# massquantity/LibRecommender

Hardware: AMD Instinct MI355X
Metric: train samples/sec (higher is better)
Workload: dtype f32 (split-bf16 x6 MFMA products, f32 accumulate); 1 GPU; DeepFM ranking train step, 1M users x 1M items x 200 sparse fields (10,000,200 sparse rows), embed_size=64, hidden=(128,64,32), Zipf(1.05) ids; per_gpu_batch=16384, global_batch=16384, fields=202, embed_size=64, table_rows=12000202, parallelism=single, launch=one hipGraph replay per step

## Files before the change

### include/libreco_hip.h

```cpp
#ifndef LIBRECO_HIP_H_
#define LIBRECO_HIP_H_

#include <stddef.h>
#include <stdint.h>

#ifdef __cplusplus
extern "C" {
#endif

#define LR_OK 0
#define LR_EINVAL (-1)
#define LR_ESHAPE (-2)
#define LR_EWORKSPACE (-3)

typedef void* lr_stream_t;

const char* lr_strerror(int code);
int lr_abi_version(void);
int lr_graph_foreign_nodes(void* graph, int* n_nodes_out);

int lr_embed_gather_f32(const float* table, int64_t V, int K, const int32_t* idx,
                        int64_t n, float* out, lr_stream_t stream);

#define LR_COMBINER_SUM 0
// ... 199 lines not shown
                                float momentum, const float* gamma, const float* beta,
                                float* moving_mean, float* moving_var, float* mean, float* inv, float* s,
                                float* t, lr_stream_t stream);
int lr_deepfm_l1_fold_stats_bias_f32(const float* partial, int F, int C, int K, int64_t B, float eps,
                                     float momentum, const float* gamma, const float* beta,
                                     float* moving_mean, float* moving_var, float* mean, float* inv, float* s,
                                     float* t, const float* W, const float* b, int H1, float* bias_partial,
                                     lr_stream_t stream);
int lr_deepfm_l1_pack_scaled_f32(const float* W, const float* scale, int F, int K, int H1, float* WpA,
                                 float* WpB, const float* red_partial, int red_nblk, float* red_out,
                                 lr_stream_t stream);
int lr_deepfm_l1_fold_bias_slabs(int n_rows);
int lr_deepfm_l1_fold_bias_f32(const float* t, const float* W, const float* b, int n_rows, int H1,
                               float* partial, lr_stream_t stream);
int lr_deepfm_l1_fold_bwd_f32(const float* part, int n_slabs, int n_rows, int H1, int64_t B,
                              const float* sgz, const float* W, const float* gamma, const float* beta,
                              const float* mean, const float* inv, float* dW, float* dgamma,
                              float* dbeta, float* db, float* bn_a, float* bn_c, lr_stream_t stream);

size_t lr_adam_coef_bytes(void);
int lr_adam_coef_store(lr_adam_hp hp, void* coef_dev, lr_stream_t stream);
int lr_adam_dense_dc_f32(float* table, float* m, float* v, int64_t n, const float* grad,
                         const void* coef_dev, lr_stream_t stream);
int lr_fm_rows_adam_dc_f32(float* table, float* m, float* v, float* lin, float* lin_m, float* lin_v,
                           int64_t V, int K, const float* ge, const float* gl, const float* wp,
                           const float* bn_a, const float* bn_c, const float* lin_scale, int64_t B,
                           int F, const int32_t* seg_pos, const int32_t* seg_rows,
                           const int32_t* seg_start, const int32_t* n_seg, const void* coef_dev,
                           void* ws, size_t ws_bytes, lr_stream_t stream);
int lr_embed_scatter_adam_dc_f32(float* table, float* m, float* v, int64_t V, int K, const float* grad,
                                 const int32_t* seg_pos, const int32_t* seg_rows, const int32_t* seg_start,
                                 const int32_t* n_seg, int64_t n_max, const void* coef_dev,
                                 void* ws, size_t ws_bytes, lr_stream_t stream);
int lr_embed_scatter_adam_lin_dc_f32(float* table, float* m, float* v, int64_t V, int K, const float* grad,
                                     float* lin, float* lin_m, float* lin_v, const float* glin,
                                     const int32_t* seg_pos, const int32_t* seg_rows,
                                     const int32_t* seg_start, const int32_t* n_seg, int64_t n_max,
                                     const void* coef_dev, lr_stream_t stream);

int lr_table_colstats_f32(const float* table, int64_t V, int K, const int32_t* idx, int64_t B, int F, int C,
                          float* partial, lr_stream_t stream);
int lr_bn_remainder_f32(float* G, const float* x, const float* a, const float* c, int64_t rows,
                        int64_t rows_per_plane, int64_t period, int Kp, lr_stream_t stream);

size_t lr_segments_fields_ws_bytes(int64_t B, int F);
int lr_segments_build_fields(const int32_t* idxT, int64_t B, int F, const int32_t* field_row_start,
                             int32_t* seg_pos, int32_t* seg_rows, int32_t* seg_start,
                             int32_t* n_seg, int32_t* slotT, void* ws, size_t ws_bytes,
                             lr_stream_t stream);
int lr_segments_build_fields_runs(const int32_t* idxT, int64_t B, int F, const int32_t* field_row_start,
                                  int32_t* seg_pos, int32_t* seg_rows, int32_t* seg_start,
                                  int32_t* n_seg, int32_t* slotT, int32_t* runT, void* ws, size_t ws_bytes,
                                  lr_stream_t stream);

size_t lr_owner_partition_ws_bytes(int64_t n_max, int W);
int lr_owner_partition_i32(const int32_t* rows, const int32_t* n_seg, int64_t n_max, int W, int32_t* perm,
                           int32_t* send_ids, int64_t* counts, void* ws, size_t ws_bytes, lr_stream_t stream);

size_t lr_din_attn_ws_bytes(int64_t B, int L, int K, int H);
int lr_din_attn_path(int K, int L, int backward);
int lr_din_build_ids_i32(const int32_t* users, const int32_t* items, const int32_t* sparse, int sparse_ld,
                         const int32_t* cols, int n_plain, const int32_t* seqs, const int32_t* lens, int64_t B, int L,
                         int32_t user_off, int32_t item_off, int32_t sparse_off, int32_t* ids, lr_stream_t stream);
int lr_din_attn_pool_fwd_f32(const float* item_table, int64_t V, int K,
                             const int32_t* item, const int32_t* seq, const int32_t* len,
                             int64_t B, int L, const float* W1, const float* b1,
                             const float* W2, const float* b2, int H, float* out,
                             float* attn, float* hid , int32_t* order_out ,
                             lr_stream_t stream);
int lr_din_attn_pool_bwd_f32(const float* item_table, int64_t V, int K,
                             const int32_t* item, const int32_t* seq, const int32_t* len,
                             int64_t B, int L, const float* W1, const float* b1,
                             const float* W2, const float* b2, int H, const float* attn,
                             const float* gout, float* gq, float* gkey, float* gW1,
                             float* gb1, float* gW2, float* gb2, void* ws, size_t ws_bytes,
                             lr_stream_t stream);
int lr_din_attn_pool_bwd_parts_f32(const float* item_table, int64_t V, int K,
                                   const int32_t* item, const int32_t* seq, const int32_t* len,
                                   int64_t B, int L, const float* W1, const float* b1,
                                   const float* W2, const float* b2, int H, const float* attn,
                                   const float* gout, float* gq, float* gkey, float* gW1,
                                   float* gb1, float* gW2, float* gb2, void* ws, size_t ws_bytes,
                                   int parts, int keep_pad_rows, const float* hid ,
                                   const int32_t* order , lr_stream_t stream);
int lr_din_attn_dense_fwd_f32(const float* q, const float* keys, int K, const int32_t* len,
                              int64_t B, int L, const float* W1, const float* b1,
                              const float* W2, const float* b2, int H, float* out,
                              float* attn, lr_stream_t stream);
int lr_din_attn_dense_bwd_f32(const float* q, const float* keys, int K, const int32_t* len,
                              int64_t B, int L, const float* W1, const float* b1,
                              const float* W2, const float* b2, int H, const float* attn,
                              const float* gout, float* gq, float* gkey, float* gW1,
                              float* gb1, float* gW2, float* gb2, void* ws, size_t ws_bytes,
                              lr_stream_t stream);

void lr_score_topk_test_mute(int ut);
size_t lr_score_topk_ws_bytes(int64_t B, int64_t N, int D, int k);
int lr_score_topk_f32(const float* users, int64_t B, const float* items, int64_t N, int D,
                      const int64_t* consumed_ptr ,
                      const int32_t* consumed_idx, const uint8_t* filter_flag ,
                      int k, int64_t item_base, float* out_scores ,
                      int64_t* out_ids , void* ws, size_t ws_bytes,
                      lr_stream_t stream);
int lr_score_topk_sb_f32(const float* users, int64_t B, const float* items, int64_t N, int D,
                         const int64_t* consumed_ptr, const int32_t* consumed_idx, const uint8_t* filter_flag,
                         int k, int64_t item_base, float* out_scores, int64_t* out_ids, void* ws, size_t ws_bytes,
// ... 323 lines not shown
```

### librecommender_amd/_lib.py

```python
from __future__ import annotations

import ctypes as C
import os
from pathlib import Path

LIB_PATH = Path(__file__).resolve().parent / "lib" / "liblibreco_hip.so"

LR_OK, LR_EINVAL, LR_ESHAPE, LR_EWORKSPACE = 0, -1, -2, -3
ABI_VERSION = 25

COMBINERS = {"sum": 0, "mean": 1, "sqrtn": 2}


class AdamHP(C.Structure):

    _fields_ = [
        ("lr", C.c_double),
        ("beta1", C.c_double),
        ("beta2", C.c_double),
        ("eps", C.c_double),
        ("weight_decay", C.c_double),
        ("step", C.c_int32),
        ("tf_style", C.c_int32),
    ]
# ... 82 lines not shown
                                    _i64, _p, _p, _p, _p, _u32, _f32, _int, _p]),
    "lr_mlp_first_bwd_f32": (_int, [_p, _p, _p, _p, _p, _p, _p, _i64, _int, _p, _p, _p]),
    "lr_reduce_partials_f32": (_int, [_p, _int, _i64, _i64, _p, _p]),
    "lr_deepfm_l1_fold_stats_f32": (_int, [_p, _int, _int, _int, _i64, _f32, _f32, _p, _p, _p, _p, _p, _p, _p, _p, _p]),
    "lr_deepfm_l1_pack_scaled_f32": (_int, [_p, _p, _int, _int, _int, _p, _p, _p, _int, _p, _p]),
    "lr_deepfm_l1_fold_stats_bias_f32": (_int, [_p, _int, _int, _int, _i64, _f32, _f32, _p, _p, _p, _p, _p, _p, _p, _p, _p, _p, _int,
                                                _p, _p]),
    "lr_deepfm_l1_fold_bias_slabs": (_int, [_int]),
    "lr_deepfm_l1_fold_bias_f32": (_int, [_p, _p, _p, _int, _int, _p, _p]),
    "lr_deepfm_l1_fold_bwd_f32": (_int, [_p, _int, _int, _int, _i64, _p, _p, _p, _p, _p, _p, _p, _p, _p, _p, _p, _p, _p]),
    "lr_fm_field_stats_slots_f32": (_int, [_p, _int, _p, _p, _p, _p, _int, _int, _p, _p, _p, _p]),
    "lr_fm_rows_grad_f32": (_int, [_p, _p, _i64, _int, _p, _p, _p, _p, _p, _p, _i64, _int, _p, _p, _p, _p, _p, _p, _p, _p,
                                   _sz, _p]),
    "lr_fm_rows_grad_compact_f32": (_int, [_p, _p, _i64, _int, _p, _p, _p, _p, _p, _p, _i64, _int, _p, _p, _p, _p, _p, _p, _p,
                                           _sz, _p]),
    "lr_adam_dense_rows_f32": (_int, [_p, _p, _p, _p, _p, _p, _i64, _int, _p, _p, _p, _p, _i64, _p, AdamHP, _p]),
    "lr_adam_dense_rows_dc_f32": (_int, [_p, _p, _p, _p, _p, _p, _i64, _int, _p, _p, _p, _p, _i64, _p, _p, _p]),
    "lr_spmm_csr_ws_bytes": (_sz, [_i64, _i64, _int]),
    "lr_spmm_csr_bucketed_f32": (_int, [_p, _p, _p, _i64, _i64, _p, _int, _p, _p, _p, _sz, _int, _p]),
    "lr_spmm_csr_masked_f32": (_int, [_p, _p, _p, _i64, _i64, _p, _int, _p, _p, _p, _p, _p, _sz, _int, _p]),
    "lr_bitmap_ids_i32": (_int, [_p, _i64, _i64, _p, _int, _p]),
    "lr_row_slots_i32": (_int, [_p, _p, _i64, _p, _int, _p]),
    "lr_spmm_csr_adam_f32": (_int, [_p, _p, _p, _i64, _i64, _p, _int, _p, _p, _p, _p, _p, _p, _f32, AdamHP, _p, _sz, _int, _p]),
    "lr_din_build_ids_i32": (_int, [_p, _p, _p, _int, _p, _int, _p, _p, _i64, _int, _int, _int, _int, _p, _p]),
    "lr_softmax_ce_supported": (_int, [_i64, _i64, _int]),
    "lr_softmax_ce_fwd_ws_bytes": (_sz, [_i64, _i64, _int, _int]),
    "lr_softmax_ce_fwd_f32": (_int, [_p, _i64, _p, _i64, _int, _p, _p, _p, _i64, _p, _p, _p, _p, _sz, _int, _p]),
    "lr_softmax_ce_bwd_cols_f32": (_int, [_p, _i64, _p, _i64, _int, _p, _p, _p, _i64, _p, _p, _p, _int, _p]),
    "lr_reduce_job_bytes": (_sz, []),
    "lr_reduce_partials_multi_f32": (_int, [_p, _int, _i64, _p]),
    "lr_pair_mlp_supported": (_int, [_int, _int]),
    "lr_pair_mlp_f32": (_int, [_p, _i64, _p, _i64, _int, _p, _p, _int, _p, _f32, _p, _i64, _int, _p]),
    "lr_pair_mlp_sb_f32": (_int, [_p, _i64, _p, _i64, _int, _p, _p, _int, _p, _f32, _p, _i64, _int, _p]),
    "lr_score_topk_test_mute": (None, [_int]),
    "lr_mfma_f32_probe": (_int, [_int, _int, _p, _p]),
    "lr_probe_occupy": (_int, [_int, _sz, _i64, _p]),
    "lr_clock_probe": (_int, [_p, _p]),
    "lr_clock_probe_slots": (_int, []),
    "lr_mlp_tail3_resident_blocks": (_int, []),
    "lr_adam_coef_bytes": (_sz, []),
    "lr_adam_coef_store": (_int, [AdamHP, _p, _p]),
    "lr_adam_dense_dc_f32": (_int, [_p, _p, _p, _i64, _p, _p, _p]),
    "lr_fm_rows_adam_dc_f32": (_int, [_p, _p, _p, _p, _p, _p, _i64, _int, _p, _p, _p, _p, _p, _p, _i64,
                                      _int, _p, _p, _p, _p, _p, _p, _sz, _p]),
    "lr_embed_scatter_adam_dc_f32": (_int, [_p, _p, _p, _i64, _int, _p, _p, _p, _p, _p, _i64, _p, _p, _sz, _p]),
    "lr_embed_scatter_adam_lin_dc_f32": (_int, [_p, _p, _p, _i64, _int, _p, _p, _p, _p, _p, _p, _p, _p, _p, _i64, _p, _p]),
    "lr_table_colstats_f32": (_int, [_p, _i64, _int, _p, _i64, _int, _int, _p, _p]),
    "lr_bn_remainder_f32": (_int, [_p, _p, _p, _p, _i64, _i64, _i64, _int, _p]),
    "lr_csr_laplacian_ws_bytes": (_sz, [_i64]),
    "lr_csr_laplacian_build": (_int, [_p, _p, _i64, _i64, _i64, _p, _p, _p, _p, _p, _p, _sz, _p]),
    "lr_segments_fields_ws_bytes": (_sz, [_i64, _int]),
    "lr_segments_build_fields": (_int, [_p, _i64, _int, _p, _p, _p, _p, _p, _p, _p, _sz, _p]),
    "lr_segments_build_fields_runs": (_int, [_p, _i64, _int, _p, _p, _p, _p, _p, _p, _p, _p, _sz, _p]),
    "lr_owner_partition_ws_bytes": (_sz, [_i64, _int]),
    "lr_owner_partition_i32": (_int, [_p, _p, _i64, _int, _p, _p, _p, _p, _sz, _p]),
    "lr_din_attn_ws_bytes": (_sz, [_i64, _int, _int, _int]),
    "lr_din_attn_path": (_int, [_int, _int, _int]),
    "lr_din_attn_pool_fwd_f32": (_int, [_p, _i64, _int, _p, _p, _p, _i64, _int, _p, _p, _p, _p,
                                        _int, _p, _p, _p, _p, _p]),
    "lr_din_attn_pool_bwd_f32": (_int, [_p, _i64, _int, _p, _p, _p, _i64, _int, _p, _p, _p, _p,
                                        _int, _p, _p, _p, _p, _p, _p, _p, _p, _p, _sz, _p]),
    "lr_din_attn_pool_bwd_parts_f32": (_int, [_p, _i64, _int, _p, _p, _p, _i64, _int, _p, _p, _p, _p,
                                              _int, _p, _p, _p, _p, _p, _p, _p, _p, _p, _sz, _int, _int, _p, _p, _p]),
    "lr_din_attn_dense_fwd_f32": (_int, [_p, _p, _int, _p, _i64, _int, _p, _p, _p, _p, _int, _p,
                                         _p, _p]),
    "lr_din_attn_dense_bwd_f32": (_int, [_p, _p, _int, _p, _i64, _int, _p, _p, _p, _p, _int, _p,
                                         _p, _p, _p, _p, _p, _p, _p, _p, _sz, _p]),
    "lr_score_topk_ws_bytes": (_sz, [_i64, _i64, _int, _int]),
    "lr_score_topk_f32": (_int, [_p, _i64, _p, _i64, _int, _p, _p, _p, _int, _i64, _p, _p, _p,
                                 _sz, _p]),
    "lr_score_topk_sb_f32": (_int, [_p, _i64, _p, _i64, _int, _p, _p, _p, _int, _i64, _p, _p, _p,
                                 _sz, _p]),
    "lr_score_topk_filter_kp": (_int, [_int]),
    "lr_score_topk_filter_ws_bytes": (_sz, [_i64, _i64, _int, _int]),
    "lr_score_topk_filter_f32": (_int, [_p, _i64, _p, _i64, _int, _p, _p, _p, _int, _i64, _p, _p, _p,
                                        _sz, _int, _int, _p, _p]),
    "lr_topk_merge_f32": (_int, [_p, _p, _int, _i64, _int, _p, _p, _p]),
    "lr_ivf_supported": (_int, [_i64, _i64, _int, _int, _int, _int]),
    "lr_ivf_search_ws_bytes": (_sz, [_i64, _i64, _int, _int, _int, _int]),
    "lr_ivf_build_ws_bytes": (_sz, [_i64, _int]),
    "lr_ivf_centroids_ws_bytes": (_sz, [_i64, _int]),
    "lr_ivf_assign_f32": (_int, [_p, _i64, _p, _int, _int, _p, _p, _p]),
    "lr_ivf_build_lists": (_int, [_p, _i64, _int, _p, _p, _p, _sz, _p]),
    "lr_ivf_centroids_f32": (_int, [_p, _i64, _int, _p, _p, _i64, _int, _p, _p, _sz, _p]),
    "lr_ivf_search_f32": (_int, [_p, _i64, _p, _int, _p, _p, _p, _i64, _int, _p, _p, _p, _int, _int, _p, _p, _p, _sz, _p]),
    "lr_spmm_csr_f32": (_int, [_p, _p, _p, _i64, _p, _int, _p, _p, _p]),
    "lr_pair_dot_f32": (_int, [_p, _i64, _p, _i64, _int, _p, _p, _i64, _p, _p]),
    "lr_als_supported": (_int, [_int]),
    "lr_als_plan_params": (_int, [_int, _p]),
    "lr_als_ws_bytes": (_sz, [_i64, _int]),
    "lr_als_gram_ws_bytes": (_sz, [_i64, _int]),
    "lr_als_gram_f32": (_int, [_p, _i64, _int, _f32, _int, _p, _p, _sz, _p]),
    "lr_als_half_sweep_f32": (_int, [_p, _p, _p, _i64, _p, _p, _int, _p, _int, _int, _int, _p, _i64, _i64, _i64, _i64,
                                     _p, _p, _sz, _int, _p]),
    "lr_cf_sim_tile_cols": (_int, []),
    "lr_cf_sim_ws_bytes": (_sz, []),
    "lr_cf_sim_f32": (_int, [_p, _p, _p, _p, _p, _p, _i64, _p, _p, _int, _int, _p, _p, _p, _i64, _int, _p, _p, _p, _p,
                             _p, _sz, _p]),
    "lr_cf_select_max": (_int, []),
    "lr_cf_topk_f32": (_int, [_p, _p, _p, _i64, _i64, _p, _p, _p, _p]),
    "lr_cf_recommend_ws_bytes": (_sz, [_i64, _i64]),
    "lr_cf_recommend_f32": (_int, [_p, _i64, _int, _p, _p, _p, _p, _p, _p, _i64, _i64, _p, _p, _int, _i64, _p, _p, _p,
                                   _p, _p, _p, _sz, _p]),
    "lr_cf_predict_f32": (_int, [_p, _p, _i64, _p, _p, _p, _p, _p, _p, _i64, _int, _f32, _f32, _f32, _p, _p, _p]),
    "lr_cf_pair_state_f32": (_int, [_p, _p, _p, _p, _p, _p, _i64, _p, _p, _p, _i64, _int, _p, _p, _p, _p, _p, _p, _sz, _p]),
    "lr_cf_sumsq_f32": (_int, [_p, _p, _i64, _int, _p, _p]),
# ... 144 lines not shown
```

### librecommender_amd/csrc/segments.hip

```cpp
#include <cstring>

#include <rocprim/rocprim.hpp>

#include "common.hpp"

namespace lr {

__global__ __launch_bounds__(kBlock) void seg_keys_kernel(const int32_t* __restrict__ idx,
                                                          int64_t n, uint32_t V,
                                                          uint32_t* __restrict__ keys) {
  const int64_t stride = static_cast<int64_t>(gridDim.x) * kBlock;
  for (int64_t i = static_cast<int64_t>(blockIdx.x) * kBlock + threadIdx.x; i < n; i += stride) {
    const int32_t id = idx[i];
    keys[i] = (id >= 0 && static_cast<uint32_t>(id) < V) ? static_cast<uint32_t>(id) : V;
  }
}

__global__ __launch_bounds__(kBlock) void seg_heads_kernel(const uint32_t* __restrict__ keys,
                                                           int64_t n, uint32_t V,
                                                           int32_t* __restrict__ heads,
                                                           int32_t* __restrict__ n_seg,
                                                           int32_t* __restrict__ seg_start) {
  const int64_t stride = static_cast<int64_t>(gridDim.x) * kBlock;
  const int64_t t0 = static_cast<int64_t>(blockIdx.x) * kBlock + threadIdx.x;
  if (t0 == 0) {
    n_seg[0] = 0;
    seg_start[0] = 0;
  }
  for (int64_t i = t0; i < n; i += stride) {
    const uint32_t k = keys[i];
    heads[i] = (k < V && (i == 0 || keys[i - 1] != k)) ? 1 : 0;
  }
}

__global__ __launch_bounds__(kBlock) void seg_emit_kernel(
    const uint32_t* __restrict__ keys, const int32_t* __restrict__ rank, int64_t n, uint32_t V,
    const int32_t* __restrict__ seg_pos, int32_t* __restrict__ seg_rows,
    int32_t* __restrict__ seg_start, int32_t* __restrict__ n_seg,
    int32_t* __restrict__ pos_to_seg) {
  const int64_t stride = static_cast<int64_t>(gridDim.x) * kBlock;
  for (int64_t i = static_cast<int64_t>(blockIdx.x) * kBlock + threadIdx.x; i < n; i += stride) {
    const uint32_t k = keys[i];
    if (k >= V) {
      if (pos_to_seg != nullptr) pos_to_seg[seg_pos[i]] = -1;
      continue;
    }
    const int32_t r = rank[i];
    if (pos_to_seg != nullptr) pos_to_seg[seg_pos[i]] = r - 1;
    if (i == 0 || keys[i - 1] != k) {
      seg_rows[r - 1] = static_cast<int32_t>(k);
      seg_start[r - 1] = static_cast<int32_t>(i);
    }
    if (i == n - 1 || keys[i + 1] >= V) {
      seg_start[r] = static_cast<int32_t>(i + 1);
      n_seg[0] = r;
    }
  }
}

static inline size_t align_up(size_t x, size_t a = 256) { return (x + a - 1) / a * a; }

static inline int key_bits(int64_t V) {
  int bits = 1;
  while (bits < 32 && (static_cast<uint64_t>(1) << bits) <= static_cast<uint64_t>(V)) ++bits;
  return bits;
}

struct SegWs {
  uint32_t* keys_in;
  uint32_t* keys_out;
  int32_t* rank;
  void* prim;
  size_t prim_bytes;
};

static inline size_t seg_fixed_bytes(int64_t n) {
  return align_up(static_cast<size_t>(n) * 4) * 3;
}

constexpr int kFS = 16384;
constexpr int kSortThreads = 1024;
constexpr int kSortWaves = kSortThreads / 64;
constexpr int kFSE = kFS / kSortThreads;
constexpr int kFSW = kFS / kSortWaves;
constexpr uint32_t kKeyInvalid = 0xFFFFFFFFu;

__device__ __forceinline__ uint64_t match_digit(uint32_t d) {
  uint64_t mask = ~0ull;
#pragma unroll
  for (int k = 0; k < 8; ++k) {
    const bool bit = (d >> k) & 1u;
    const uint64_t bk = __ballot(bit);
    mask &= bit ? bk : ~bk;
  }
  return mask;
}

__global__ __launch_bounds__(kSortThreads) void seg_field_sort_kernel(
    const int32_t* __restrict__ idxT, int B, const int32_t* __restrict__ frs,
    uint64_t* __restrict__ sorted, int32_t* __restrict__ fcount) {
  extern __shared__ __attribute__((aligned(16))) char smem[];
  uint64_t* buf = reinterpret_cast<uint64_t*>(smem);
  int* cnt = reinterpret_cast<int*>(buf + kFS);
  int* wsum = cnt + kSortWaves * 256;
  const int f = blockIdx.x;
  const int tid = threadIdx.x, wid = tid >> 6, lane = tid & 63;
  const int32_t lo = frs[f], hi = frs[f + 1];
  const uint64_t lt = (1ull << lane) - 1ull;
  const int32_t* col = idxT + static_cast<int64_t>(f) * B;
  int bits = 0;
  while (bits < 32 && ((1ull << bits) - 1ull) < static_cast<uint64_t>(hi > lo ? hi - lo : 0)) ++bits;
  const int n_pass = (bits + 7) / 8;

  uint64_t x[kFSE];
#pragma unroll
  for (int s = 0; s < kFSE; ++s) {
    const int p = wid * kFSW + s * 64 + lane;
    const int32_t id = p < B ? col[p] : -1;
    const bool ok = id >= lo && id < hi;
    const uint32_t key = ok ? static_cast<uint32_t>(id - lo) : kKeyInvalid;
    x[s] = (static_cast<uint64_t>(key) << 32) | static_cast<uint32_t>(p);
  }

  int* my = cnt + wid * 256;
  for (int pass = 0; pass < n_pass; ++pass) {
    const int shift = 32 + 8 * pass;
    for (int i = tid; i < kSortWaves * 256; i += kSortThreads) cnt[i] = 0;
    __syncthreads();
#pragma unroll
    for (int s = 0; s < kFSE; ++s) {
      const uint32_t d = static_cast<uint32_t>(x[s] >> shift) & 255u;
      const uint64_t mk = match_digit(d);
      if ((mk & lt) == 0ull)
        __hip_atomic_fetch_add(my + d, __popcll(mk), __ATOMIC_RELAXED, __HIP_MEMORY_SCOPE_WORKGROUP);
    }
    __syncthreads();
    int tot = 0, inc = 0;
    if (tid < 256) {
#pragma unroll
      for (int w = 0; w < kSortWaves; ++w) tot += cnt[w * 256 + tid];
      inc = tot;
#pragma unroll
      for (int o = 1; o < 64; o <<= 1) {
        const int y = __shfl_up(inc, o);
        if (lane >= o) inc += y;
      }
      if (lane == 63) wsum[wid] = inc;
    }
    __syncthreads();
    if (tid < 256) {
      int run = inc - tot;
      for (int w = 0; w < wid; ++w) run += wsum[w];
#pragma unroll
      for (int w = 0; w < kSortWaves; ++w) {
        const int c = cnt[w * 256 + tid];
        cnt[w * 256 + tid] = run;
        run += c;
      }
    }
    __syncthreads();
#pragma unroll
    for (int s = 0; s < kFSE; ++s) {
      uint32_t d = static_cast<uint32_t>(x[s] >> shift) & 255u;
      asm volatile("" : "+v"(d));
      const uint64_t mk = match_digit(d);
      const int leader = __ffsll(static_cast<long long>(mk)) - 1;
      int old = 0;
      if (lane == leader)
        old = __hip_atomic_fetch_add(my + d, __popcll(mk), __ATOMIC_RELAXED, __HIP_MEMORY_SCOPE_WORKGROUP);
      old = __shfl(old, leader);
      buf[old + __popcll(mk & lt)] = x[s];
      if ((s & 3) == 3) __builtin_amdgcn_sched_barrier(0);
    }
    __syncthreads();
#pragma unroll
    for (int s = 0; s < kFSE; ++s) x[s] = buf[wid * kFSW + s * 64 + lane];
  }
  if (n_pass == 0) {
#pragma unroll
    for (int s = 0; s < kFSE; ++s) buf[wid * kFSW + s * 64 + lane] = x[s];
  }
  __syncthreads();

  int nv = 0, nh = 0;
  uint64_t* dst = sorted + static_cast<int64_t>(f) * B;
#pragma unroll
  for (int s = 0; s < kFSE; ++s) {
    const int i = wid * kFSW + s * 64 + lane;
    const uint32_t key = static_cast<uint32_t>(x[s] >> 32);
    const bool valid = key != kKeyInvalid;
    const bool head = valid && (i == 0 || static_cast<uint32_t>(buf[i > 0 ? i - 1 : 0] >> 32) != key);
    nv += __popcll(__ballot(valid));
    nh += __popcll(__ballot(head));
    if (i < B) dst[i] = x[s];
  }
  __syncthreads();
  if (lane == 0) { wsum[wid * 2] = nv; wsum[wid * 2 + 1] = nh; }
  __syncthreads();
  if (tid == 0) {
    int tv = 0, th = 0;
    for (int w = 0; w < kSortWaves; ++w) { tv += wsum[2 * w]; th += wsum[2 * w + 1]; }
    fcount[2 * f] = tv;
    fcount[2 * f + 1] = th;
  }
}

constexpr int kEmitThreads = 1024;
constexpr int kEmitWaves = kEmitThreads / 64;

__global__ __launch_bounds__(kEmitThreads) void seg_field_emit_kernel(
    const uint64_t* __restrict__ sorted, const int32_t* __restrict__ fcount, int B, int F,
    const int32_t* __restrict__ frs, int32_t* __restrict__ seg_pos, int32_t* __restrict__ seg_rows,
    int32_t* __restrict__ seg_start, int32_t* __restrict__ n_seg, int32_t* __restrict__ slotT,
    int32_t* __restrict__ runT) {
  __shared__ int red[2][kEmitWaves];
  __shared__ int wh[kEmitWaves];
  const int f = blockIdx.x;
  const int tid = threadIdx.x, wid = tid >> 6, lane = tid & 63;
  const uint64_t lt = (1ull << lane) - 1ull;
  int bv = 0, bh = 0;
  for (int g = tid; g < f; g += kEmitThreads) { bv += fcount[2 * g]; bh += fcount[2 * g + 1]; }
#pragma unroll
  for (int o = 32; o > 0; o >>= 1) { bv += __shfl_xor(bv, o); bh += __shfl_xor(bh, o); }
  if (lane == 0) { red[0][wid] = bv; red[1][wid] = bh; }
  __syncthreads();
  int base_v = 0, base_h = 0;
#pragma unroll
  for (int w = 0; w < kEmitWaves; ++w) { base_v += red[0][w]; base_h += red[1][w]; }
  const int nv = fcount[2 * f];
  const int32_t lo = frs[f];
  const uint64_t* src = sorted + static_cast<int64_t>(f) * B;
  const int chunk = ((B + kEmitWaves - 1) / kEmitWaves + 63) / 64 * 64;
  const int i0 = wid * chunk, i1 = (i0 + chunk) < B ? (i0 + chunk) : B;
  auto is_head = [&](int i, uint32_t key) {
    return i < nv && (i == 0 || static_cast<uint32_t>(src[i - 1] >> 32) != key);
// ... 183 lines not shown
  const size_t a = align_up(static_cast<size_t>(n) * 4);
  SegWs w;
  w.keys_in = reinterpret_cast<uint32_t*>(p);
  w.keys_out = reinterpret_cast<uint32_t*>(p + a);
  w.rank = reinterpret_cast<int32_t*>(p + 2 * a);
  w.prim = p + 3 * a;
  w.prim_bytes = ws_bytes - 3 * a;

  const uint32_t Vu = static_cast<uint32_t>(V);
  const int grid = grid_for(n, kBlock);
  hipLaunchKernelGGL(seg_keys_kernel, dim3(grid), dim3(kBlock), 0, s, idx, n, Vu, w.keys_in);

  const int bits = key_bits(V);
  size_t need = 0;
  hipError_t e = hipSuccess;
  if (n <= kRsMaxN) {
    const size_t hist_bytes = align_up((static_cast<size_t>((n + kRsKPB - 1) / kRsKPB) + 1) * 256 * 4);
    if (hist_bytes + a > w.prim_bytes) return LR_EWORKSPACE;
    const int rc = own_radix_sort(w.keys_in, w.keys_out, seg_pos, reinterpret_cast<uint32_t*>(static_cast<char*>(w.prim) + hist_bytes),
                                  w.rank, static_cast<int32_t*>(w.prim), n, bits, s);
    if (rc != LR_OK) return rc;
  } else {
    rocprim::counting_iterator<int32_t> iota(0);
    e = rocprim::radix_sort_pairs(nullptr, need, w.keys_in, w.keys_out, iota, seg_pos, static_cast<size_t>(n), 0u,
                                  static_cast<unsigned>(bits), s);
    if (e != hipSuccess) return static_cast<int>(e);
    if (need > w.prim_bytes) return LR_EWORKSPACE;
    e = rocprim::radix_sort_pairs(w.prim, need, w.keys_in, w.keys_out, iota, seg_pos, static_cast<size_t>(n), 0u,
                                  static_cast<unsigned>(bits), s);
    if (e != hipSuccess) return static_cast<int>(e);
  }

  hipLaunchKernelGGL(seg_heads_kernel, dim3(grid), dim3(kBlock), 0, s, w.keys_out, n, Vu,
                     w.rank, n_seg, seg_start);
  need = 0;
  e = rocprim::inclusive_scan(nullptr, need, w.rank, w.rank, static_cast<size_t>(n),
                              rocprim::plus<int32_t>(), s);
  if (e != hipSuccess) return static_cast<int>(e);
  if (need > w.prim_bytes) return LR_EWORKSPACE;
  e = rocprim::inclusive_scan(w.prim, need, w.rank, w.rank, static_cast<size_t>(n),
                              rocprim::plus<int32_t>(), s);
  if (e != hipSuccess) return static_cast<int>(e);

  hipLaunchKernelGGL(seg_emit_kernel, dim3(grid), dim3(kBlock), 0, s, w.keys_out, w.rank, n,
                     Vu, seg_pos, seg_rows, seg_start, n_seg, pos_to_seg);
  return launch_status();
}

extern "C" size_t lr_segments_fields_ws_bytes(int64_t B, int F) {
  if (B < 0 || F < 1) return 0;
  return align_up(static_cast<size_t>(B) * F * 8) + align_up(static_cast<size_t>(F) * 8);
}

static int build_fields_impl(const int32_t* idxT, int64_t B, int F, const int32_t* field_row_start, int32_t* seg_pos,
                             int32_t* seg_rows, int32_t* seg_start, int32_t* n_seg, int32_t* slotT, int32_t* runT, void* ws,
                             size_t ws_bytes, lr_stream_t stream) {
  LR_CHECK_ARG(B >= 1 && F >= 1);
  LR_CHECK_ARG(idxT && field_row_start && seg_pos && seg_rows && seg_start && n_seg && ws);
  if (B > kFS || B * F >= (int64_t(1) << 31)) return LR_ESHAPE;
  if (ws_bytes < lr_segments_fields_ws_bytes(B, F)) return LR_EWORKSPACE;
  hipStream_t s = as_stream(stream);
  uint64_t* sorted = static_cast<uint64_t*>(ws);
  int32_t* fcount = reinterpret_cast<int32_t*>(static_cast<char*>(ws) + align_up(static_cast<size_t>(B) * F * 8));
  const size_t lds = static_cast<size_t>(kFS) * 8 + kSortWaves * 256 * 4 + kSortWaves * 2 * 4;
  static bool attr_set = false;
  if (!attr_set) {
    hipError_t e = hipFuncSetAttribute(reinterpret_cast<const void*>(seg_field_sort_kernel),
                                       hipFuncAttributeMaxDynamicSharedMemorySize, static_cast<int>(lds));
    if (e != hipSuccess) return static_cast<int>(e);
    attr_set = true;
  }
  hipLaunchKernelGGL(seg_field_sort_kernel, dim3(F), dim3(kSortThreads), lds, s, idxT, static_cast<int>(B),
                     field_row_start, sorted, fcount);
  hipLaunchKernelGGL(seg_field_emit_kernel, dim3(F), dim3(kEmitThreads), 0, s, sorted, fcount,
                     static_cast<int>(B), F, field_row_start, seg_pos, seg_rows, seg_start, n_seg, slotT, runT);
  return launch_status();
}

extern "C" int lr_segments_build_fields(const int32_t* idxT, int64_t B, int F, const int32_t* field_row_start,
                                        int32_t* seg_pos, int32_t* seg_rows, int32_t* seg_start, int32_t* n_seg,
                                        int32_t* slotT, void* ws, size_t ws_bytes, lr_stream_t stream) {
  return build_fields_impl(idxT, B, F, field_row_start, seg_pos, seg_rows, seg_start, n_seg, slotT, nullptr, ws, ws_bytes,
                           stream);
}

extern "C" int lr_segments_build_fields_runs(const int32_t* idxT, int64_t B, int F, const int32_t* field_row_start,
                                             int32_t* seg_pos, int32_t* seg_rows, int32_t* seg_start, int32_t* n_seg,
                                             int32_t* slotT, int32_t* runT, void* ws, size_t ws_bytes, lr_stream_t stream) {
  LR_CHECK_ARG(runT != nullptr);
  return build_fields_impl(idxT, B, F, field_row_start, seg_pos, seg_rows, seg_start, n_seg, slotT, runT, ws, ws_bytes,
                           stream);
}

constexpr int kOwnChunk = 1024;
constexpr int kOwnMaxW = 64;

template <bool kPlace>
__device__ __forceinline__ void owner_chunk(const int32_t* __restrict__ rows, int n, int W, int chunk, int (*cnt)[4][kOwnMaxW],
                                            int* my_owner, int* my_rank) {
  const int tid = threadIdx.x, wid = tid >> 6, lane = tid & 63;
  const uint64_t lt = (1ull << lane) - 1ull;
#pragma unroll
  for (int it = 0; it < 4; ++it) {
    const int i = chunk * kOwnChunk + it * kBlock + tid;
    const int o = i < n ? static_cast<int>(static_cast<uint32_t>(rows[i]) % static_cast<uint32_t>(W)) : -1;
    int rank = 0;
    for (int w = 0; w < W; ++w) {
      const uint64_t mk = __ballot(o == w);
      if (o == w) rank = __popcll(mk & lt);
      if (lane == 0) cnt[it][wid][w] = __popcll(mk);
    }
    if (kPlace) { my_owner[it] = o; my_rank[it] = rank; }
  }
}

__global__ __launch_bounds__(kBlock) void owner_count_kernel(const int32_t* __restrict__ rows, const int32_t* __restrict__ n_seg,
                                                             int W, int32_t* __restrict__ chunk_cnt) {
  __shared__ int cnt[4][4][kOwnMaxW];
  const int n = n_seg[0];
  const int chunk = blockIdx.x;
  if (chunk * kOwnChunk >= n) {
    for (int w = threadIdx.x; w < W; w += kBlock) chunk_cnt[static_cast<int64_t>(chunk) * W + w] = 0;
    return;
  }
  owner_chunk<false>(rows, n, W, chunk, cnt, nullptr, nullptr);
  __syncthreads();
  for (int w = threadIdx.x; w < W; w += kBlock) {
    int t = 0;
#pragma unroll
// ... 97 lines not shown
```

### librecommender_amd/ops.py

```python
from __future__ import annotations

import os

from dataclasses import dataclass
from typing import NamedTuple, Optional

import torch

from . import _lib
from ._lib import AdamHP, COMBINERS, check


def _stream() -> int:
    return torch.cuda.current_stream().cuda_stream


class KernelTimer:

    def __init__(self):
        self.names = set()
        self.events = {}

    def enable(self, *names):
        self.names = set(names)
# ... 138 lines not shown
        nbytes = _lib.load().lr_segments_ws_bytes(self.n_max, self.V)
        self.ws = torch.empty(nbytes, dtype=torch.uint8, device=device)
        self.pos = torch.empty(self.n_max, dtype=torch.int32, device=device)
        self.rows = torch.empty(self.n_max, dtype=torch.int32, device=device)
        self.start = torch.empty(self.n_max + 1, dtype=torch.int32, device=device)
        self.n_seg = torch.zeros(1, dtype=torch.int32, device=device)
        self.slots = None
        self._long_ws = {}

    def long_ws(self, K: int) -> torch.Tensor:
        ws = self._long_ws.get(K)
        if ws is None:
            ws = self._long_ws[K] = torch.empty(max(_lib.load().lr_embed_scatter_ws_bytes(self.n_max, K), 256),
                                                dtype=torch.uint8, device=self.device)
        return ws

    def hist_ws(self, K: int) -> torch.Tensor:
        ws = self._long_ws.get(("hist", K))
        if ws is None:
            ws = self._long_ws[("hist", K)] = torch.empty(max(_lib.load().lr_svdpp_hist_grad_ws_bytes(self.n_max, K), 256),
                                                          dtype=torch.uint8, device=self.device)
        return ws

    def ftrl_ws(self) -> torch.Tensor:
        ws = self._long_ws.get("ftrl")
        if ws is None:
            ws = self._long_ws["ftrl"] = torch.empty(max(_lib.load().lr_ftrl_rows_ws_bytes(self.n_max), 256),
                                                     dtype=torch.uint8, device=self.device)
        return ws

    def build(self, idx: torch.Tensor, want_slots: bool = False) -> Segments:
        _req(idx, torch.int32, "idx")
        n = idx.numel()
        if n > self.n_max:
            raise ValueError(f"idx has {n} entries, builder was sized for {self.n_max}")
        if want_slots and self.slots is None:
            self.slots = torch.empty(self.n_max, dtype=torch.int32, device=self.device)
        _call("lr_segments_build", _ptr(idx), n, self.V, _ptr(self.pos), _ptr(self.rows),
                                            _ptr(self.start), _ptr(self.n_seg),
                                            _ptr(self.slots) if want_slots else None, _ptr(self.ws),
                                            self.ws.numel(), _stream())
        seg = Segments(self.pos, self.rows, self.start, self.n_seg, n, self.V, owner=self)
        seg.slots = self.slots[:n] if want_slots else None
        return seg


def build_segments(idx: torch.Tensor, V: int) -> Segments:
    return SegmentBuilder(max(idx.numel(), 1), V, idx.device).build(idx)


class FieldSegmentBuilder:

    MAX_B = 16384

    def __init__(self, B_max: int, F: int, V: int, device: torch.device, want_runs: bool = False):
        self.B_max, self.F, self.V, self.device = int(B_max), int(F), int(V), device
        n = self.B_max * self.F
        self.ws = torch.empty(_lib.load().lr_segments_fields_ws_bytes(self.B_max, self.F), dtype=torch.uint8, device=device)
        self.pos = torch.empty(n, dtype=torch.int32, device=device)
        self.rows = torch.empty(n, dtype=torch.int32, device=device)
        self.start = torch.empty(n + 1, dtype=torch.int32, device=device)
        self.n_seg = torch.zeros(1, dtype=torch.int32, device=device)
        self.slotT = torch.empty((self.F, self.B_max), dtype=torch.int32, device=device)
        self.runT = torch.empty((self.F, self.B_max), dtype=torch.int32, device=device) if want_runs else None

    def build(self, idxT: torch.Tensor, field_row_start: torch.Tensor) -> Segments:
        _req(idxT, torch.int32, "idxT", 2)
        _req(field_row_start, torch.int32, "field_row_start", 1)
        F, B = idxT.shape
        if F != self.F or B > self.B_max or field_row_start.numel() != F + 1:
            raise ValueError("idxT does not match this builder")
        cut = (lambda t: t if B == self.B_max else t.view(-1)[: F * B].view(F, B))
        slotT = cut(self.slotT)
        seg = Segments(self.pos, self.rows, self.start, self.n_seg, B * F, self.V)
        if self.runT is None:
            _call("lr_segments_build_fields", _ptr(idxT), B, F, _ptr(field_row_start), _ptr(self.pos), _ptr(self.rows),
                  _ptr(self.start), _ptr(self.n_seg), _ptr(slotT), _ptr(self.ws), self.ws.numel(), _stream())
        else:
            seg.runT = cut(self.runT)
            _call("lr_segments_build_fields_runs", _ptr(idxT), B, F, _ptr(field_row_start), _ptr(self.pos), _ptr(self.rows),
                  _ptr(self.start), _ptr(self.n_seg), _ptr(slotT), _ptr(seg.runT), _ptr(self.ws), self.ws.numel(), _stream())
        seg.slotT = slotT
        return seg


class OwnerPartition:

    def __init__(self, n_max: int, W: int, device: torch.device):
        self.n_max, self.W = int(n_max), int(W)
        self.ws = torch.empty(max(_lib.load().lr_owner_partition_ws_bytes(self.n_max, self.W), 256), dtype=torch.uint8, device=device)
        self.perm = torch.empty(self.n_max, dtype=torch.int32, device=device)
        self.send_ids = torch.empty(self.n_max, dtype=torch.int32, device=device)
        self.counts = torch.zeros(self.W + 1, dtype=torch.int64, device=device)

    def run(self, rows: torch.Tensor, n_seg: torch.Tensor):
        _req(rows, torch.int32, "rows", 1)
        _req(n_seg, torch.int32, "n_seg", 1)
        if rows.numel() > self.n_max:
            raise ValueError("rows exceed this partition's capacity")
        _call("lr_owner_partition_i32", _ptr(rows), _ptr(n_seg), rows.numel(), self.W, _ptr(self.perm), _ptr(self.send_ids),
              _ptr(self.counts), _ptr(self.ws), self.ws.numel(), _stream())
        return self.perm, self.send_ids, self.counts


def idx_transpose(idx: torch.Tensor, out: Optional[torch.Tensor] = None) -> torch.Tensor:
    _req(idx, torch.int32, "idx", 2)
    B, F = idx.shape
    if out is None:
        out = torch.empty((F, B), dtype=torch.int32, device=idx.device)
    _call("lr_idx_transpose_i32", _ptr(idx), B, F, _ptr(out), _stream())
    return out


def din_build_ids(users, items, sparse, cols, seqs, lens, user_off: int, item_off: int, sparse_off: int,
                  out: torch.Tensor) -> torch.Tensor:
    for t_, n_ in ((users, "users"), (items, "items"), (seqs, "seqs"), (lens, "lens"), (out, "out")):
        _req(t_, torch.int32, n_)
    B, L = seqs.shape
    n_plain = 0
    if sparse is not None:
        _req(sparse, torch.int32, "sparse", 2)
        n_plain = int(cols.numel()) if cols is not None else sparse.shape[1]
        if cols is not None:
            _req(cols, torch.int32, "cols", 1)
    if out.numel() != (2 + n_plain + 2 + L) * B or not seqs.is_contiguous() or (sparse is not None and not sparse.is_contiguous()):
        raise ValueError("`out` must hold (2 + n_plain + 2 + L) * B ids; seqs / sparse contiguous")
    _call("lr_din_build_ids_i32", _ptr(users), _ptr(items), _ptr(sparse), sparse.shape[1] if sparse is not None else 0,
          _ptr(cols), n_plain, _ptr(seqs), _ptr(lens), B, L, int(user_off), int(item_off), int(sparse_off), _ptr(out), _stream())
    return out


def _din_order(order, B):
    if order is not None and (order.dtype != torch.int32 or not order.is_contiguous() or order.numel() != B):
        raise ValueError("order must be a contiguous int32 tensor of B elements")
    return order


def embed_segment_sum(grad: torch.Tensor, seg: Segments) -> torch.Tensor:
    _req(grad, torch.float32, "grad")
    K = grad.shape[-1]
    if grad.numel() != seg.n * K:
        raise ValueError("grad rows must match the segmented index count")
    grows = torch.zeros((max(seg.n, 1), K), dtype=torch.float32, device=grad.device)
    ws = seg.long_ws(K)
    _call("lr_embed_segment_sum_f32", _ptr(grad), K, _ptr(seg.pos), _ptr(seg.start), _ptr(seg.n_seg), seg.n, _ptr(grows),
          _ptr(ws), 0 if ws is None else ws.numel(), _stream())
    return grows


def embed_scatter_add(table: torch.Tensor, grad: torch.Tensor, seg: Segments, alpha: float = 1.0) -> None:
    _req(table, torch.float32, "table", 2)
    _req(grad, torch.float32, "grad")
    V, K = table.shape
    if grad.numel() != seg.n * K or V != seg.V:
        raise ValueError("shape mismatch")
    ws = seg.long_ws(K)
    _call("lr_embed_scatter_add_f32", _ptr(table), V, K, _ptr(grad), _ptr(seg.pos), _ptr(seg.rows), _ptr(seg.start),
          _ptr(seg.n_seg), seg.n, float(alpha), _ptr(ws), 0 if ws is None else ws.numel(), _stream())


def embed_scatter_adam(table: torch.Tensor, m: torch.Tensor, v: torch.Tensor, grad: torch.Tensor,
                       seg: Segments, hp) -> None:
# ... 2694 lines not shown
```

Before: 6.582 million samples/s.

## Fuse per-field counting into idx transpose and emit segments inside sort kernel

```diff
diff --git a/include/libreco_hip.h b/include/libreco_hip.h
--- a/include/libreco_hip.h
+++ b/include/libreco_hip.h
@@ -275,6 +275,8 @@
                                   int32_t* seg_pos, int32_t* seg_rows, int32_t* seg_start,
                                   int32_t* n_seg, int32_t* slotT, int32_t* runT, void* ws, size_t ws_bytes,
                                   lr_stream_t stream);
+int lr_idx_transpose_count_i32(const int32_t* idx, int64_t B, int F, const int32_t* field_row_start,
+                               int64_t max_field_rows, int32_t* idxT, void* ws, size_t ws_bytes, lr_stream_t stream);
 
 size_t lr_owner_partition_ws_bytes(int64_t n_max, int W);
 int lr_owner_partition_i32(const int32_t* rows, const int32_t* n_seg, int64_t n_max, int W, int32_t* perm,
diff --git a/librecommender_amd/_lib.py b/librecommender_amd/_lib.py
--- a/librecommender_amd/_lib.py
+++ b/librecommender_amd/_lib.py
@@ -158,6 +158,7 @@
     "lr_segments_fields_ws_bytes": (_sz, [_i64, _int]),
     "lr_segments_build_fields": (_int, [_p, _i64, _int, _p, _p, _p, _p, _p, _p, _p, _sz, _p]),
     "lr_segments_build_fields_runs": (_int, [_p, _i64, _int, _p, _p, _p, _p, _p, _p, _p, _p, _sz, _p]),
+    "lr_idx_transpose_count_i32": (_int, [_p, _i64, _int, _p, _i64, _p, _p, _sz, _p]),
     "lr_owner_partition_ws_bytes": (_sz, [_i64, _int]),
     "lr_owner_partition_i32": (_int, [_p, _p, _i64, _int, _p, _p, _p, _p, _sz, _p]),
     "lr_din_attn_ws_bytes": (_sz, [_i64, _int, _int, _int]),
diff --git a/librecommender_amd/csrc/segments.hip b/librecommender_amd/csrc/segments.hip
--- a/librecommender_amd/csrc/segments.hip
+++ b/librecommender_amd/csrc/segments.hip
@@ -1,4 +1,5 @@
 #include <cstring>
+#include <mutex>
 
 #include <rocprim/rocprim.hpp>
 
@@ -96,9 +97,59 @@
   return mask;
 }
 
+constexpr int kCountThreads = 1024;
+constexpr int kCountWaves = kCountThreads / 64;
+constexpr int64_t kCountMaxRows = (int64_t(160) * 1024 - 256) * 8;
+
+__global__ __launch_bounds__(kCountThreads) void seg_field_count_kernel(
+    const int32_t* __restrict__ idx, int B, int F, const int32_t* __restrict__ frs, uint32_t cap_rows,
+    int32_t* __restrict__ idxT, int32_t* __restrict__ fcount) {
+  extern __shared__ __attribute__((aligned(16))) char smem[];
+  uint32_t* bm = reinterpret_cast<uint32_t*>(smem);
+  __shared__ int red[2][kCountWaves];
+  const int per = (F + 7) / 8;
+  const int f = static_cast<int>(blockIdx.x % 8u) * per + static_cast<int>(blockIdx.x / 8u);
+  if (f >= F) return;
+  const int tid = threadIdx.x, wid = tid >> 6, lane = tid & 63;
+  const int32_t lo = frs[f], hi = frs[f + 1];
+  const uint32_t range = hi > lo ? static_cast<uint32_t>(hi - lo) : 0u;
+  const uint32_t rows = range < cap_rows ? range : cap_rows;
+  const int nwords = static_cast<int>((rows + 31u) / 32u);
+  for (int w = tid; w < nwords; w += kCountThreads) bm[w] = 0u;
+  __syncthreads();
+  int nv = 0;
+  int32_t* dst = idxT + static_cast<int64_t>(f) * B;
+  const int32_t* src = idx + f;
+#pragma unroll 4
+  for (int b = tid; b < B; b += kCountThreads) {
+    const int32_t id = src[static_cast<int64_t>(b) * F];
+    dst[b] = id;
+    const bool ok = id >= lo && id < hi;
+    nv += ok ? 1 : 0;
+    const uint32_t r = static_cast<uint32_t>(id - lo);
+    if (ok && r < rows) atomicOr(&bm[r >> 5], 1u << (r & 31u));
+  }
+  __syncthreads();
+  int nh = 0;
+  for (int w = tid; w < nwords; w += kCountThreads) nh += __popc(bm[w]);
+#pragma unroll
+  for (int o = 32; o > 0; o >>= 1) { nv += __shfl_xor(nv, o); nh += __shfl_xor(nh, o); }
+  if (lane == 0) { red[0][wid] = nv; red[1][wid] = nh; }
+  __syncthreads();
+  if (tid == 0) {
+    int tv = 0, th = 0;
+    for (int w = 0; w < kCountWaves; ++w) { tv += red[0][w]; th += red[1][w]; }
+    fcount[2 * f] = tv;
+    fcount[2 * f + 1] = th;
+  }
+}
+
+template <bool kEmit>
 __global__ __launch_bounds__(kSortThreads) void seg_field_sort_kernel(
-    const int32_t* __restrict__ idxT, int B, const int32_t* __restrict__ frs,
-    uint64_t* __restrict__ sorted, int32_t* __restrict__ fcount) {
+    const int32_t* __restrict__ idxT, int B, int F, const int32_t* __restrict__ frs,
+    uint64_t* __restrict__ sorted, int32_t* __restrict__ fcount, int32_t* __restrict__ seg_pos,
+    int32_t* __restrict__ seg_rows, int32_t* __restrict__ seg_start, int32_t* __restrict__ n_seg,
+    int32_t* __restrict__ slotT, int32_t* __restrict__ runT) {
   extern __shared__ __attribute__((aligned(16))) char smem[];
   uint64_t* buf = reinterpret_cast<uint64_t*>(smem);
   int* cnt = reinterpret_cast<int*>(buf + kFS);
@@ -181,6 +232,87 @@
     for (int s = 0; s < kFSE; ++s) buf[wid * kFSW + s * 64 + lane] = x[s];
   }
   __syncthreads();
+
+  if constexpr (kEmit) {
+    int bv = 0, bh = 0;
+    for (int g = tid; g < f; g += kSortThreads) { bv += fcount[2 * g]; bh += fcount[2 * g + 1]; }
+#pragma unroll
+    for (int o = 32; o > 0; o >>= 1) { bv += __shfl_xor(bv, o); bh += __shfl_xor(bh, o); }
+    int* red = cnt;
+    uint64_t* hbm = reinterpret_cast<uint64_t*>(cnt + kSortWaves * 4) + wid * kFSE;
+    int nv = 0, nh = 0;
+#pragma unroll 1
+    for (int s = 0; s < kFSE; ++s) {
+      const int i = wid * kFSW + s * 64 + lane;
+      const uint32_t key = static_cast<uint32_t>(buf[i] >> 32);
+      const bool valid = key != kKeyInvalid;
+      const bool head = valid && (i == 0 || static_cast<uint32_t>(buf[i > 0 ? i - 1 : 0] >> 32) != key);
+      const uint64_t hb = __ballot(head);
+      if (lane == 0) hbm[s] = hb;
+      nv += __popcll(__ballot(valid));
+      nh += __popcll(hb);
+    }
+    if (lane == 0) {
+      red[wid * 4] = bv; red[wid * 4 + 1] = bh; red[wid * 4 + 2] = nv; red[wid * 4 + 3] = nh;
+    }
+    __syncthreads();
+    int base_v = 0, base_h = 0, tot_v = 0, tot_h = 0, run = 0;
+#pragma unroll
+    for (int w = 0; w < kSortWaves; ++w) {
+      base_v += red[w * 4];
+      base_h += red[w * 4 + 1];
+      tot_v += red[w * 4 + 2];
+      const int h = red[w * 4 + 3];
+      tot_h += h;
+      run += w < wid ? h : 0;
+    }
+    run += base_h;
+#pragma unroll 1
+    for (int s = 0; s < kFSE; ++s) {
+      const int i = wid * kFSW + s * 64 + lane;
+      const uint64_t e = buf[i];
+      const uint32_t key = static_cast<uint32_t>(e >> 32);
+      const uint32_t p = static_cast<uint32_t>(e);
+      const bool valid = key != kKeyInvalid;
+      const uint64_t hb = hbm[s];
+      const bool h = (hb >> lane) & 1ull;
+      const int rn = valid ? run + __popcll(hb & (lt | (1ull << lane))) - 1 : -1;
+      if (valid) seg_pos[base_v + i] = static_cast<int32_t>(p) * F + f;
+      if (h) {
+        seg_rows[rn] = lo + static_cast<int32_t>(key);
+        seg_start[rn] = base_v + i;
+      }
+      buf[i] = (static_cast<uint64_t>(static_cast<uint32_t>(rn)) << 32) | p;
+      run += __popcll(hb);
+    }
+    if (f == F - 1 && tid == 0) {
+      seg_start[base_h + tot_h] = base_v + tot_v;
+      n_seg[0] = base_h + tot_h;
+    }
+    __syncthreads();
+#pragma unroll
+    for (int s = 0; s < kFSE; ++s) x[s] = buf[wid * kFSW + s * 64 + lane];
+    __syncthreads();
+    int32_t* slot_l = reinterpret_cast<int32_t*>(buf);
+    int32_t* run_l = slot_l + kFS;
+#pragma unroll
+    for (int s = 0; s < kFSE; ++s) {
+      const int i = wid * kFSW + s * 64 + lane;
+      const int p = static_cast<int>(static_cast<uint32_t>(x[s]));
+      const int rn = static_cast<int>(static_cast<uint32_t>(x[s] >> 32));
+      if (p < B) {
+        slot_l[p] = rn >= 0 ? base_v + i : -1;
+        run_l[p] = rn;
+      }
+    }
+    __syncthreads();
+    const int64_t fB = static_cast<int64_t>(f) * B;
+    for (int b = tid; b < B; b += kSortThreads) {
+      if (slotT != nullptr) slotT[fB + b] = slot_l[b];
+      if (runT != nullptr) runT[fB + b] = run_l[b];
+    }
+    return;
+  }
 
   int nv = 0, nh = 0;
   uint64_t* dst = sorted + static_cast<int64_t>(f) * B;
@@ -470,6 +602,30 @@
   return align_up(static_cast<size_t>(B) * F * 8) + align_up(static_cast<size_t>(F) * 8);
 }
 
+static inline int32_t* fields_fcount(void* ws, int64_t B, int F) {
+  return reinterpret_cast<int32_t*>(static_cast<char*>(ws) + align_up(static_cast<size_t>(B) * F * 8));
+}
+
+struct FieldCounts {
+  const int32_t* idxT;
+  const int32_t* frs;
+  void* ws;
+  int64_t B;
+  int F;
+  hipStream_t stream;
+};
+static std::mutex g_counted_mu;
+static FieldCounts g_counted{nullptr, nullptr, nullptr, 0, 0, nullptr};
+
+static bool take_counted(const FieldCounts& c) {
+  std::lock_guard<std::mutex> g(g_counted_mu);
+  if (g_counted.idxT == nullptr || g_counted.ws != c.ws) return false;
+  const bool same = g_counted.idxT == c.idxT && g_counted.frs == c.frs && g_counted.B == c.B && g_counted.F == c.F &&
+                    g_counted.stream == c.stream;
+  g_counted.idxT = nullptr;
+  return same;
+}
+
 static int build_fields_impl(const int32_t* idxT, int64_t B, int F, const int32_t* field_row_start, int32_t* seg_pos,
                              int32_t* seg_rows, int32_t* seg_start, int32_t* n_seg, int32_t* slotT, int32_t* runT, void* ws,
                              size_t ws_bytes, lr_stream_t stream) {
@@ -479,20 +635,59 @@
   if (ws_bytes < lr_segments_fields_ws_bytes(B, F)) return LR_EWORKSPACE;
   hipStream_t s = as_stream(stream);
   uint64_t* sorted = static_cast<uint64_t*>(ws);
-  int32_t* fcount = reinterpret_cast<int32_t*>(static_cast<char*>(ws) + align_up(static_cast<size_t>(B) * F * 8));
+  int32_t* fcount = fields_fcount(ws, B, F);
   const size_t lds = static_cast<size_t>(kFS) * 8 + kSortWaves * 256 * 4 + kSortWaves * 2 * 4;
   static bool attr_set = false;
   if (!attr_set) {
-    hipError_t e = hipFuncSetAttribute(reinterpret_cast<const void*>(seg_field_sort_kernel),
+    hipError_t e = hipFuncSetAttribute(reinterpret_cast<const void*>(seg_field_sort_kernel<false>),
                                        hipFuncAttributeMaxDynamicSharedMemorySize, static_cast<int>(lds));
+    if (e == hipSuccess)
+      e = hipFuncSetAttribute(reinterpret_cast<const void*>(seg_field_sort_kernel<true>),
+                              hipFuncAttributeMaxDynamicSharedMemorySize, static_cast<int>(lds));
     if (e != hipSuccess) return static_cast<int>(e);
     attr_set = true;
   }
-  hipLaunchKernelGGL(seg_field_sort_kernel, dim3(F), dim3(kSortThreads), lds, s, idxT, static_cast<int>(B),
-                     field_row_start, sorted, fcount);
+  const FieldCounts now{idxT, field_row_start, ws, B, F, s};
+  if (take_counted(now)) {
+    hipLaunchKernelGGL(seg_field_sort_kernel<true>, dim3(F), dim3(kSortThreads), lds, s, idxT, static_cast<int>(B), F,
+                       field_row_start, nullptr, fcount, seg_pos, seg_rows, seg_start, n_seg, slotT, runT);
+    return launch_status();
+  }
+  hipLaunchKernelGGL(seg_field_sort_kernel<false>, dim3(F), dim3(kSortThreads), lds, s, idxT, static_cast<int>(B), F,
+                     field_row_start, sorted, fcount, nullptr, nullptr, nullptr, nullptr, nullptr, nullptr);
   hipLaunchKernelGGL(seg_field_emit_kernel, dim3(F), dim3(kEmitThreads), 0, s, sorted, fcount,
                      static_cast<int>(B), F, field_row_start, seg_pos, seg_rows, seg_start, n_seg, slotT, runT);
   return launch_status();
+}
+
+extern "C" int lr_idx_transpose_count_i32(const int32_t* idx, int64_t B, int F, const int32_t* field_row_start,
+                                          int64_t max_field_rows, int32_t* idxT, void* ws, size_t ws_bytes,
+                                          lr_stream_t stream) {
+  LR_CHECK_ARG(B >= 1 && F >= 1 && max_field_rows >= 0);
+  LR_CHECK_ARG(idx && field_row_start && idxT && ws);
+  if (B > kFS || B * F >= (int64_t(1) << 31) || max_field_rows > kCountMaxRows) return LR_ESHAPE;
+  if (ws_bytes < lr_segments_fields_ws_bytes(B, F)) return LR_EWORKSPACE;
+  hipStream_t s = as_stream(stream);
+  const size_t lds = align_up(static_cast<size_t>((max_field_rows + 31) / 32) * 4);
+  static size_t attr_lds = 0;
+  {
+    std::lock_guard<std::mutex> g(g_counted_mu);
+    g_counted.idxT = nullptr;
+    if (lds > attr_lds) {
+      hipError_t e = hipFuncSetAttribute(reinterpret_cast<const void*>(seg_field_count_kernel),
+                                         hipFuncAttributeMaxDynamicSharedMemorySize, static_cast<int>(lds));
+      if (e != hipSuccess) return static_cast<int>(e);
+      attr_lds = lds;
+    }
+  }
+  hipLaunchKernelGGL(seg_field_count_kernel, dim3(8 * ((F + 7) / 8)), dim3(kCountThreads), lds, s, idx, static_cast<int>(B), F,
+                     field_row_start, static_cast<uint32_t>(max_field_rows), idxT, fields_fcount(ws, B, F));
+  const int rc = launch_status();
+  if (rc == LR_OK) {
+    std::lock_guard<std::mutex> g(g_counted_mu);
+    g_counted = FieldCounts{idxT, field_row_start, ws, B, F, s};
+  }
+  return rc;
 }
 
 extern "C" int lr_segments_build_fields(const int32_t* idxT, int64_t B, int F, const int32_t* field_row_start,
diff --git a/librecommender_amd/ops.py b/librecommender_amd/ops.py
--- a/librecommender_amd/ops.py
+++ b/librecommender_amd/ops.py
@@ -214,9 +214,11 @@
 class FieldSegmentBuilder:
 
     MAX_B = 16384
+    BITMAP_MAX_ROWS = (160 * 1024 - 256) * 8
 
     def __init__(self, B_max: int, F: int, V: int, device: torch.device, want_runs: bool = False):
         self.B_max, self.F, self.V, self.device = int(B_max), int(F), int(V), device
+        self._ranges = None
         n = self.B_max * self.F
         self.ws = torch.empty(_lib.load().lr_segments_fields_ws_bytes(self.B_max, self.F), dtype=torch.uint8, device=device)
         self.pos = torch.empty(n, dtype=torch.int32, device=device)
@@ -243,7 +245,20 @@
             _call("lr_segments_build_fields_runs", _ptr(idxT), B, F, _ptr(field_row_start), _ptr(self.pos), _ptr(self.rows),
                   _ptr(self.start), _ptr(self.n_seg), _ptr(slotT), _ptr(seg.runT), _ptr(self.ws), self.ws.numel(), _stream())
         seg.slotT = slotT
+        if getattr(idxT, "_lr_field_plan", None) is None:
+            self._adopt(idxT, field_row_start)
         return seg
+
+    def _adopt(self, idxT: torch.Tensor, field_row_start: torch.Tensor) -> None:
+        if torch.cuda.is_current_stream_capturing():
+            return
+        r = self._ranges
+        if r is None or r[0] is not field_row_start or r[1] != field_row_start._version:
+            edges = field_row_start.cpu().to(torch.int64)
+            widest = int((edges[1:] - edges[:-1]).max())
+            r = self._ranges = (field_row_start, field_row_start._version, widest)
+        if 0 <= r[2] <= self.BITMAP_MAX_ROWS:
+            idxT._lr_field_plan = (self,) + r
 
 
 class OwnerPartition:
@@ -270,6 +285,13 @@
     B, F = idx.shape
     if out is None:
         out = torch.empty((F, B), dtype=torch.int32, device=idx.device)
+    plan = getattr(out, "_lr_field_plan", None)
+    if plan is not None:
+        fb, frs, version, widest = plan
+        if fb.F == F and 1 <= B <= min(fb.B_max, fb.MAX_B) and frs._version == version and frs.numel() == F + 1:
+            _call("lr_idx_transpose_count_i32", _ptr(idx), B, F, _ptr(frs), widest, _ptr(out), _ptr(fb.ws), fb.ws.numel(),
+                  _stream())
+            return out
     _call("lr_idx_transpose_i32", _ptr(idx), B, F, _ptr(out), _stream())
     return out
 
```

After: 6.624 million samples/s, median of 6. No clear change (+0.6%).
